# Pixie8888/R3DFSSeg

Measured on NVIDIA B200. Metric: MPTI episodes/s (2-way 5-shot, 2048 pts), higher is better.
Workload: dtype f32

## Files before the change

### r3dfsseg_b200/csrc/common.cuh

```cuda
#pragma once
#include <cuda_runtime.h>
#include <stdint.h>
#include <math.h>

#include "../../include/r3dfs.h"

#define R3DFS_FEAT_DIM 192
#define R3DFS_EC_WIDTH 64

extern thread_local long long r3dfs_launches;

#ifdef R3DFS_AB_SWITCHES
#include <stdlib.h>
#define R3DFS_GETENV(name) getenv(name)
#else
#define R3DFS_GETENV(name) ((const char*)nullptr)
#endif

#define R3DFS_CHECK_LAUNCH()                       \
  do {                                             \
    cudaError_t e__ = cudaGetLastError();          \
    if (e__ != cudaSuccess) return (int)e__;       \
    ++r3dfs_launches;                              \
  } while (0)
// ... 6 lines not shown
};

#define R3DFS_TRY(expr)                            \
  do {                                             \
    int rc__ = (expr);                             \
    if (rc__ != 0) return rc__;                    \
  } while (0)

static inline size_t align_up(size_t x, size_t a) { return (x + a - 1) / a * a; }

__host__ __device__ inline int lp_rowcap(int k) { return ((2 * k + 3) & ~3) + 4; }
__host__ __device__ inline int64_t lp_pack_groups(int64_t nn, int k) {
  return (nn * (int64_t)(2 * k) * 2 / 5 + 64 * nn + 63) / 64 * 64;
}
static inline size_t lp_solver_scratch_bytes(size_t G, size_t nn, int k) {
  return G * 16 * (4 + 32 * 3 * 2 + 3 * 1024 * 2) * 4 + 256 + 4 * G * (1 + nn) + 256 +
         (8 + 16) * G * (size_t)lp_pack_groups(nn, k) + 512;
}

struct WsBump {
  char* base;
  size_t cap;
  size_t off;
  __host__ WsBump(void* p, size_t c) : base((char*)p), cap(c), off(0) {}
  template <typename T>
  __host__ T* take(size_t n) {
    off = align_up(off, 256);
    T* r = (T*)(base + off);
    off += n * sizeof(T);
    return r;
  }
  __host__ bool ok() const { return off <= cap; }
// ... 92 lines not shown
```

### r3dfsseg_b200/csrc/lp.cu

```cuda
#include <cooperative_groups.h>

#include <stdlib.h>

#include "common.cuh"
#include "lp.cuh"

namespace cg = cooperative_groups;

#define GD_BM 128
#define GD_BN 64
#define GD_BK 16

template <int ROWS, int KC>
__device__ __forceinline__ void lp_load_tile_T(float* __restrict__ dst,
                                               const float* __restrict__ src, int ld, int64_t row0,
                                               int64_t rows_end, int k0, int k_end) {
  constexpr int KG = KC / 8;
  constexpr int PAIRS = (ROWS / 4) * KG;
  const int lane = threadIdx.x & 31, w = threadIdx.x >> 5;
  const int nw = blockDim.x >> 5;
  const int r_lo = lane & 3, k_lo = lane >> 2;
  for (int p = w; p < PAIRS; p += nw) {
    int kg = p % KG, rg = p / KG;
    int row = 4 * rg + r_lo, kk = 8 * kg + k_lo;
// ... 754 lines not shown
#pragma unroll
  for (int r = 0; r < 8; ++r) {
    const int t = 32 * r + lane;
    if (t < L) {
      src[t] = key[r];
      val[t] = w[r];
    }
  }
}

__global__ __launch_bounds__(256) void merge_rows_kernel(
    const int32_t* __restrict__ nbr, const float* __restrict__ sim,
    const int32_t* __restrict__ in_ptr, const int32_t* __restrict__ in_src,
    const float* __restrict__ in_w, const uint8_t* __restrict__ valid, int nn, int k,
    int32_t* __restrict__ cursor, int32_t* __restrict__ rowptr, int32_t* __restrict__ rowlen,
    uint16_t* __restrict__ mcol, float* __restrict__ mval) {
  extern __shared__ __align__(16) unsigned char s_raw[];
  const int g = blockIdx.y, wi = threadIdx.x >> 5, lane = threadIdx.x & 31;
  const int i = blockIdx.x * 8 + wi;
  int* s_idx = reinterpret_cast<int*>(s_raw) + wi * k;
  float* s_val = reinterpret_cast<float*>(s_raw) + 8 * k + wi * k;
  if (i >= nn) return;
  const int64_t vb = (int64_t)g * nn;
  if (!valid[vb + i]) {
    if (lane == 0) {
      rowptr[vb + i] = 0;
      rowlen[vb + i] = 0;
    }
    return;
  }
  const int64_t ob = (vb + i) * k;
  for (int t = lane; t < k; t += 32) {
    s_idx[t] = nbr[ob + t];
    s_val[t] = sim[ob + t];
  }
  __syncwarp();
  const int32_t* ptr = in_ptr + (int64_t)g * (nn + 1);
  const int64_t ib = vb * k;
  const int e0 = ptr[i], e1 = ptr[i + 1];
  int keep = 0;
  for (int t0 = e0; t0 < e1; t0 += 32) {
    const int t = t0 + lane;
// ... 4 lines not shown
      while (lo < hi) {
        const int mid = (lo + hi) >> 1;
        if (s_idx[mid] < s) lo = mid + 1; else hi = mid;
      }
      kp = !(lo < k && s_idx[lo] == s);
    }
    keep += __popc(__ballot_sync(0xffffffffu, kp));
  }
  const int total = k + keep;
  const int padded = (total + 3) & ~3;
  int start = 0;
  if (lane == 0) start = atomicAdd(&cursor[g], padded);
  start = __shfl_sync(0xffffffffu, start, 0);
  const int64_t mb = vb * lp_rowcap(k) + start;
  int run = 0;
  for (int t0 = e0; t0 < e1; t0 += 32) {
    const int t = t0 + lane;
    bool kp = false;
    int s = 0;
    float wv = 0.f;
    if (t < e1) {
      s = in_src[ib + t];
      wv = in_w[ib + t];
      int lo = 0, hi = k;
      while (lo < hi) {
        const int mid = (lo + hi) >> 1;
        if (s_idx[mid] < s) lo = mid + 1; else hi = mid;
      }
      if (lo < k && s_idx[lo] == s) s_val[lo] += wv; else kp = true;
    }
    const unsigned bal = __ballot_sync(0xffffffffu, kp);
    if (kp) {
      const int pos = k + run + __popc(bal & ((1u << lane) - 1));
      mcol[mb + pos] = (uint16_t)s;
      mval[mb + pos] = wv;
    }
    run += __popc(bal);
  }
  __syncwarp();
  for (int t = lane; t < k; t += 32) {
    mcol[mb + t] = (uint16_t)s_idx[t];
    mval[mb + t] = s_val[t];
  }
  if (lane < padded - total) {
    mcol[mb + total + lane] = 0;
    mval[mb + total + lane] = 0.f;
  }
  if (lane == 0) {
    rowptr[vb + i] = start;
    rowlen[vb + i] = total;
  }
}

__global__ __launch_bounds__(256) void degree_merged_kernel(const int32_t* __restrict__ rowptr,
                                                            const int32_t* __restrict__ rowlen,
                                                            const float* __restrict__ mval, int nn,
                                                            int k, float* __restrict__ dinv) {
  const int g = blockIdx.y;
  const int i = blockIdx.x * 8 + (threadIdx.x >> 5);
  if (i >= nn) return;
  const int lane = threadIdx.x & 31;
  const int64_t vb = (int64_t)g * nn;
  const int L = rowlen[vb + i];
  float d = 0.f;
  if (L > 0) {
    const float* v = mval + vb * lp_rowcap(k) + rowptr[vb + i];
    for (int t = lane; t < L; t += 32) d += v[t];
    d = warp_sum(d);
    d = sqrtf(1.0f / (d + 2.220446049250313e-16f));
  }
  if (lane == 0) dinv[vb + i] = d;
}

__global__ void normalize_merged_kernel(const int32_t* __restrict__ rowptr,
                                        const int32_t* __restrict__ rowlen,
                                        const uint16_t* __restrict__ mcol, float* __restrict__ mval,
                                        const float* __restrict__ dinv, int nn, int k) {
  const int g = blockIdx.y;
  const int i = blockIdx.x * 8 + (threadIdx.x >> 5);
  if (i >= nn) return;
  const int lane = threadIdx.x & 31;
  const int64_t vb = (int64_t)g * nn;
  const int L = rowlen[vb + i];
  const float* dg = dinv + vb;
  const float di = dg[i];
  const int64_t mb = vb * lp_rowcap(k) + rowptr[vb + i];
  for (int t = lane; t < L; t += 32) mval[mb + t] = (di * mval[mb + t]) * dg[mcol[mb + t]];
}

#define CG_THREADS 1024
#define CGC_MAXT 1024
#define CG_CL_MAX 16
#define CG_MAXC 8
#define CG_MAXPASS 3
#define CG_SEGR 48
#define CG_MAXPART 1024
#define CG_TAB_HDR 4
#define CG_TAB_INTS (CG_TAB_HDR + 32 * CG_MAXPASS * 2 + CG_MAXPASS * CGC_MAXT * 2)
#define CG_PK_SMEM (4096 * 4 + 8192 * 4 * 2)

struct CgExchange {
  float slot[2][CG_CL_MAX][CG_MAXC];
};

template <int NCV>
__device__ __forceinline__ void cg_allreduce(cg::cluster_group& cluster, CgExchange* ex,
                                             float* s_warp, const float* part, int& xcnt,
                                             float* total) {
  const int tid = threadIdx.x, lane = tid & 31, w = tid >> 5;
  const int rank = cluster.block_rank(), CL = cluster.num_blocks();
  const int n_warps = blockDim.x >> 5;
  float v[NCV];
#pragma unroll
// ... 10 lines not shown
    for (int r = 0; r < CL; ++r) {
      float* dst = cluster.map_shared_rank(&ex->slot[par][rank][tid], r);
      *dst = s;
    }
  }
  cluster.sync();
#pragma unroll
  for (int c = 0; c < NCV; ++c) {
    float s = 0.f;
    for (int r = 0; r < CL; ++r) s += ex->slot[par][r][c];
    total[c] = s;
  }
  ++xcnt;
}

__global__ __launch_bounds__(256) void cg_hist_kernel(const int32_t* __restrict__ rowptr,
                                                      const int32_t* __restrict__ rowlen,
                                                      const uint8_t* __restrict__ valid,
                                                      const uint16_t* __restrict__ mcol, int nn,
                                                      int k, int32_t* __restrict__ rowmax) {
  const int g = blockIdx.y;
  const int i = blockIdx.x * 8 + (threadIdx.x >> 5);
  if (i >= nn) return;
  const int lane = threadIdx.x & 31;
  const int64_t vb = (int64_t)g * nn;
  int mx = 0;
  if (valid[vb + i]) {
    const int L = rowlen[vb + i];
    const uint16_t* c = mcol + vb * lp_rowcap(k) + rowptr[vb + i];
    int cnt[8] = {0, 0, 0, 0, 0, 0, 0, 0};
    for (int t0 = 0; t0 < L; t0 += 32) {
      const int t = t0 + lane;
      const int res = t < L ? (int)(c[t] & 7) : -1;
#pragma unroll
      for (int b = 0; b < 8; ++b) cnt[b] += __popc(__ballot_sync(0xffffffffu, res == b));
    }
#pragma unroll
    for (int b = 0; b < 8; ++b) mx = max(mx, cnt[b]);
  }
  if (lane == 0) rowmax[vb + i] = mx;
}

__global__ __launch_bounds__(1024) void cg_pack_kernel(
    const int32_t* __restrict__ rowptr, const int32_t* __restrict__ rowlen,
    const int32_t* __restrict__ rowmax, const uint16_t* __restrict__ mcol,
    const float* __restrict__ mval, int nn, int k, int64_t pk_cap, int32_t* __restrict__ tab_all,
    int32_t* __restrict__ flags, uint2* __restrict__ pcol, float4* __restrict__ pval) {
  extern __shared__ __align__(16) unsigned char pk_smem[];
  uint32_t* s_key = reinterpret_cast<uint32_t*>(pk_smem);
  int* s_pre = reinterpret_cast<int*>(s_key + 4096);
  int* s_prx = s_pre + 8192;
  __shared__ int s_scan[2][32];
  __shared__ int s_tot[2];
  __shared__ int s_rng[2];
  __shared__ int s_wtot[32], s_wbase[32];
  const int CL = gridDim.x, rank = blockIdx.x, g = blockIdx.y;
  const int tid = threadIdx.x, lane = tid & 31, w = tid >> 5;
  const int64_t vb = (int64_t)g * nn;
  const int32_t* rp = rowptr + vb;
  const int32_t* rl = rowlen + vb;
  const int32_t* rmx = rowmax + vb;
  const uint16_t* mc = mcol + vb * lp_rowcap(k);
  const float* mv = mval + vb * lp_rowcap(k);
  int32_t* tab = tab_all + (size_t)(g * CL + rank) * CG_TAB_INTS;
  for (int e = tid; e < CG_TAB_HDR + 32 * CG_MAXPASS * 2; e += 1024) tab[e] = 0;
  {
    int nseg[8], run = 0, runx = 0;
#pragma unroll
    for (int u = 0; u < 8; ++u) {
      const int i = tid * 8 + u;
      nseg[u] = i < nn ? (rmx[i] + CG_SEGR - 1) / CG_SEGR : 0;
      run += nseg[u];
      runx += nseg[u] > 1 ? nseg[u] : 0;
    }
    int inc = run, incx = runx;
#pragma unroll
    for (int o = 1; o < 32; o <<= 1) {
      const int a = __shfl_up_sync(0xffffffffu, inc, o), ax = __shfl_up_sync(0xffffffffu, incx, o);
      if (lane >= o) {
        inc += a;
        incx += ax;
      }
    }
    if (lane == 31) {
      s_scan[0][w] = inc;
      s_scan[1][w] = incx;
// ... 38 lines not shown
  const int NV = s_tot[0];
  for (int i = tid; i < nn; i += 1024) {
    const int owner = NV > 0 ? min(CL - 1, (int)((int64_t)s_pre[i] * CL / NV)) : (i * CL) / nn;
    if (owner == rank) {
      atomicMin(&s_rng[0], i);
      atomicMax(&s_rng[1], i + 1);
    }
  }
  __syncthreads();
  const int lo = min(s_rng[0], s_rng[1]), hi = s_rng[1];
  const int pre_lo = lo < nn ? s_pre[lo] : NV, prx_lo = lo < nn ? s_prx[lo] : s_tot[1];
  const int nv = (hi < nn ? s_pre[hi] : NV) - pre_lo;
  const int nx = (hi < nn ? s_prx[hi] : s_tot[1]) - prx_lo;
  const int passes = (nv + CGC_MAXT - 1) / CGC_MAXT;
  const int64_t share = pk_cap / CL;
  bool bad = passes > CG_MAXPASS || nx > CG_MAXPART || hi - lo > 8191;
  int npow = 32;
  while (npow < nv) npow <<= 1;
  if (!bad) {
    for (int i = tid; i < npow; i += 1024) s_key[i] = 0;
    __syncthreads();
    for (int i = lo + tid; i < hi; i += 1024) {
      const int mx = rmx[i];
      const int ns = (mx + CG_SEGR - 1) / CG_SEGR;
      if (ns > 255) bad = true;
      for (int sg = 0; sg < ns && sg < 256; ++sg) {
        const int ranks = min(CG_SEGR, mx - sg * CG_SEGR);
        s_key[s_pre[i] - pre_lo + sg] =
            ((uint32_t)(2 * ranks) << 21) | ((uint32_t)(i - lo) << 8) | (uint32_t)sg;
      }
    }
// ... 31 lines not shown
        run += s_wtot[q];
      }
      s_tot[0] = run;
    }
    __syncthreads();
    if (s_tot[0] > share) bad = true;
  }
  if (tid == 0) {
    tab[0] = lo;
    tab[1] = hi;
    tab[2] = bad ? 0 : passes;
    tab[3] = nx;
    if (bad) atomicOr(&flags[g], 1);
  }
  if (bad) return;
  for (int e = tid; e < CG_MAXPASS * CGC_MAXT; e += 1024) {
    const int p = e / CGC_MAXT, t = e % CGC_MAXT;
    const int i = p * CGC_MAXT + t;
    int m0 = -1, m1 = 0;
    if (p < passes && i < nv) {
      const uint32_t key = s_key[i];
      const int rloc = (int)((key >> 8) & 0x1fffu), sg = (int)(key & 0xffu);
      const int ns = (rmx[lo + rloc] + CG_SEGR - 1) / CG_SEGR;
      m0 = (rloc << 8) | sg;
      m1 = (ns << 16) | (ns > 1 ? s_prx[lo + rloc] - prx_lo : 0);
    }
    tab[CG_TAB_HDR + 32 * CG_MAXPASS * 2 + 2 * e + 0] = m0;
    tab[CG_TAB_HDR + 32 * CG_MAXPASS * 2 + 2 * e + 1] = m1;
  }
  uint2* gc = pcol + (int64_t)g * pk_cap + rank * share;
  float4* gv = pval + (int64_t)g * pk_cap + rank * share;
  int base = s_wbase[w];
  for (int p = 0; p < passes; ++p) {
    const int i0 = p * CGC_MAXT + w * 32;
    const int rounds = i0 < nv ? (int)(s_key[i0] >> 21) : 0;
    if (lane == 0) {
      tab[CG_TAB_HDR + (w * CG_MAXPASS + p) * 2 + 0] = (int)(rank * share) + base;
      tab[CG_TAB_HDR + (w * CG_MAXPASS + p) * 2 + 1] = rounds;
    }
    for (int r = 0; r < rounds; ++r) {
      const unsigned t0 = (unsigned)(lane + 4 * r);
      uint2 c2;
      c2.x = (t0 & 7u) | (((t0 + 1) & 7u) << 16);
      c2.y = ((t0 + 2) & 7u) | (((t0 + 3) & 7u) << 16);
      gc[base + r * 32 + lane] = c2;
      gv[base + r * 32 + lane] = make_float4(0.f, 0.f, 0.f, 0.f);
    }
    __syncwarp();
    uint16_t* c16 = reinterpret_cast<uint16_t*>(gc + base);
    float* v32 = reinterpret_cast<float*>(gv + base);
    int my_L = 0, my_ptr = 0, my_sg = 0;
    if (i0 + lane < nv) {
      const uint32_t key = s_key[i0 + lane];
      const int row = lo + (int)((key >> 8) & 0x1fffu);
      my_L = rl[row];
      my_ptr = rp[row];
      my_sg = (int)(key & 0xffu);
    }
    const int n_here = min(32, nv - i0);
    for (int l = 0; l < n_here; ++l) {
      const int L = __shfl_sync(0xffffffffu, my_L, l), sg = __shfl_sync(0xffffffffu, my_sg, l);
      const int ptr = __shfl_sync(0xffffffffu, my_ptr, l);
      const int r_lo = sg * CG_SEGR, r_hi = r_lo + CG_SEGR;
      const uint16_t* c = mc + ptr;
      const float* v = mv + ptr;
      int seen[8] = {0, 0, 0, 0, 0, 0, 0, 0};
      int col_n = lane < L ? (int)c[lane] : -1;
      float val_n = lane < L ? v[lane] : 0.f;
      for (int t0 = 0; t0 < L; t0 += 32) {
        const int col = col_n;
        const float val = val_n;
        const int tn = t0 + 32 + lane;
        col_n = tn < L ? (int)c[tn] : -1;
        val_n = tn < L ? v[tn] : 0.f;
        const int res = col >= 0 ? (col & 7) : -1;
        int rho = -1;
#pragma unroll
        for (int b = 0; b < 8; ++b) {
          const uint32_t m = __ballot_sync(0xffffffffu, res == b);
          if (res == b) rho = seen[b] + __popc(m & ((1u << lane) - 1));
          seen[b] += __popc(m);
        }
        if (rho >= r_lo && rho < r_hi) {
          const int step = 8 * (rho - r_lo) + ((res - l) & 7);
          const int64_t d = ((int64_t)(step >> 2) * 32 + l) * 4 + (step & 3);
          c16[d] = (uint16_t)col;
          v32[d] = val;
        }
        int done_all = 1;
#pragma unroll
        for (int b = 0; b < 8; ++b) done_all &= seen[b] >= r_hi;
        if (done_all) break;
      }
    }
    __syncwarp();
    base += rounds * 32;
  }
}

template <int NCV>
__global__ __launch_bounds__(CGC_MAXT, 1) void lp_cg_kernel(
    const int32_t* __restrict__ rowptr, const int32_t* __restrict__ rowlen,
    const uint16_t* __restrict__ mcol, const float* __restrict__ mval,
    const uint8_t* __restrict__ valid, int nn, int k,
    const float* __restrict__ Y, int nc, float alpha, float tol, int max_iter,
    float* __restrict__ Z, float* __restrict__ X, float* __restrict__ R, float* __restrict__ Pv,
    float* __restrict__ AP, int32_t* __restrict__ iters_out, float* __restrict__ resid_out,
    const int32_t* __restrict__ tab_all, const int32_t* __restrict__ flags,
    const uint2* __restrict__ pcol, const float4* __restrict__ pval, int64_t pk_cap) {
  cg::cluster_group cluster = cg::this_cluster();
  const int CL = cluster.num_blocks(), rank = cluster.block_rank();
// ... 217 lines not shown
    for (int c = 0; c < nc; ++c) Zg[(int64_t)row * nc + c] = Xg[(int64_t)row * NCV + c];
  }
  if (rank == 0 && tid == 0) {
    if (iters_out) iters_out[g] = it;
    if (resid_out) {
      float m = 0.f;
#pragma unroll
      for (int c = 0; c < NCV; ++c)
        if (bb[c] > 0.f) m = fmaxf(m, sqrtf(rs[c] / bb[c]));
      resid_out[g] = m;
    }
  }
  cluster.sync();
}

template <int NCV>
static int launch_cg(int CL, int G, size_t smem, cudaStream_t st, const int32_t* rowptr,
                     const int32_t* rowlen, const uint16_t* mcol, const float* mval,
                     const uint8_t* valid, int nn, int k, const float* Y, int nc,
                     float alpha, float tol, int max_iter, float* Z, float* X, float* R, float* P,
                     float* AP, int32_t* iters_out, float* resid_out, void* scratch,
                     size_t scratch_bytes) {
  cudaError_t e = cudaFuncSetAttribute(lp_cg_kernel<NCV>,
                                       cudaFuncAttributeMaxDynamicSharedMemorySize, 200 * 1024);
  if (e != cudaSuccess) return (int)e;
  if (CL > 8) {
    e = cudaFuncSetAttribute(lp_cg_kernel<NCV>, cudaFuncAttributeNonPortableClusterSizeAllowed, 1);
    if (e != cudaSuccess) return (int)e;
  }
  const int T = CGC_MAXT;
  smem += sizeof(float) * (size_t)CG_MAXPART * NCV;
  cudaLaunchConfig_t cfg = {};
  cfg.gridDim = dim3(CL, G, 1);
  cfg.blockDim = dim3(T, 1, 1);
  cfg.dynamicSmemBytes = smem;
  cfg.stream = st;
  cudaLaunchAttribute attr[1];
  attr[0].id = cudaLaunchAttributeClusterDimension;
  attr[0].val.clusterDim.x = CL;
  attr[0].val.clusterDim.y = 1;
  attr[0].val.clusterDim.z = 1;
  cfg.attrs = attr;
  cfg.numAttrs = 1;
  {
    int n_clusters = 0;
    e = cudaOccupancyMaxActiveClusters(&n_clusters, lp_cg_kernel<NCV>, &cfg);
    if (e != cudaSuccess || n_clusters < 1) {
      (void)cudaGetLastError();
      return -1000;
    }
  }
  const int64_t pk_cap = lp_pack_groups(nn, k);
  const size_t tab_bytes = align_up(sizeof(int32_t) * (size_t)G * CL * CG_TAB_INTS, 256);
  const size_t flg_bytes = align_up(sizeof(int32_t) * (size_t)G * (1 + nn), 256);
  const size_t col_bytes = align_up(sizeof(uint2) * (size_t)G * pk_cap, 256);
  const size_t val_bytes = align_up(sizeof(float4) * (size_t)G * pk_cap, 256);
  if (!scratch || scratch_bytes < tab_bytes + flg_bytes + col_bytes + val_bytes)
    return R3DFS_E_WORKSPACE;
  unsigned char* sp = reinterpret_cast<unsigned char*>(scratch);
  int32_t* tab = reinterpret_cast<int32_t*>(sp);
  int32_t* flags = reinterpret_cast<int32_t*>(sp + tab_bytes);
  uint2* pcol = reinterpret_cast<uint2*>(sp + tab_bytes + flg_bytes);
  float4* pval = reinterpret_cast<float4*>(sp + tab_bytes + flg_bytes + col_bytes);
  e = cudaMemsetAsync(flags, 0, sizeof(int32_t) * (size_t)G, st);
  if (e != cudaSuccess) return (int)e;
  e = cudaFuncSetAttribute(cg_pack_kernel, cudaFuncAttributeMaxDynamicSharedMemorySize, CG_PK_SMEM);
  if (e != cudaSuccess) return (int)e;
  int32_t* rowmax = flags + G;
  cg_hist_kernel<<<dim3((nn + 7) / 8, G), 256, 0, st>>>(rowptr, rowlen, valid, mcol, nn, k, rowmax);
  R3DFS_CHECK_LAUNCH();
  cg_pack_kernel<<<dim3(CL, G), 1024, CG_PK_SMEM, st>>>(rowptr, rowlen, rowmax, mcol, mval, nn, k,
                                                       pk_cap, tab, flags, pcol, pval);
  R3DFS_CHECK_LAUNCH();
  const int32_t* tabc = tab;
  const int32_t* flc = flags;
  const uint2* pc = pcol;
  const float4* pv = pval;
  e = cudaLaunchKernelEx(&cfg, lp_cg_kernel<NCV>, rowptr, rowlen, mcol, mval, valid, nn, k, Y, nc,
                         alpha, tol, max_iter, Z, X, R, P, AP, iters_out, resid_out, tabc, flc, pc,
                         pv, pk_cap);
  if (e != cudaSuccess) return (int)e;
  ++r3dfs_launches;
  return 0;
}

#define GCG_SLOT 8
#define GCG_MAX_GS 160

__device__ __forceinline__ unsigned ld_acquire_u32(const unsigned* p) {
  unsigned v;
  asm volatile("ld.acquire.gpu.global.u32 %0, [%1];" : "=r"(v) : "l"(p) : "memory");
  return v;
}

__device__ __forceinline__ void group_barrier(unsigned* cnt, unsigned& target, int GS) {
  __syncthreads();
  if (threadIdx.x == 0) {
    target += (unsigned)GS;
// ... 447 lines not shown
  if (sr) sr->mark(R3DFS_ST_SELECT, st);
  edge_sim_kernel<<<dim3((nn + 7) / 8, G), 256, 0, st>>>(F, graph_rows, row_off, nn, D, valid, nbr,
                                                        k, sigma, sim);
  R3DFS_CHECK_LAUNCH();
  if (sr) sr->mark(R3DFS_ST_SIM, st);
  return 0;
}

int launch_lp_solve(const int32_t* rowptr, const int32_t* rowlen, const uint16_t* mcol,
                    const float* mval, const uint8_t* valid, int G, int nn, int k, const float* Y,
                    int nc, float alpha, float tol, int max_iter, float* Z, float* X, float* R,
                    float* P, float* AP, int32_t* iters_out, float* resid_out, cudaStream_t st,
                    bool latency, void* scratch, size_t scratch_bytes) {
  if (nc > CG_MAXC || nc < 1 || nn > 8192) return R3DFS_E_UNSUPPORTED;
  const int ncv = nc <= 4 ? 4 : 8;
  const size_t smem_cg = sizeof(float) * (size_t)nn * ncv;
  if (smem_cg > 200 * 1024) return R3DFS_E_UNSUPPORTED;
  int rc = -1000;
  static const bool no_group = R3DFS_GETENV("R3DFS_CG_NOGROUP") != nullptr;
  if (latency && !no_group) {
    const size_t scratch_floats = (size_t)G * nn * ncv;
    rc = ncv == 4 ? launch_cg_group<4>(G, st, rowptr, rowlen, mcol, mval, valid, nn, k, Y, nc, alpha,
                                       tol, max_iter, Z, P, AP, scratch_floats, iters_out, resid_out)
                  : launch_cg_group<8>(G, st, rowptr, rowlen, mcol, mval, valid, nn, k, Y, nc, alpha,
                                       tol, max_iter, Z, P, AP, scratch_floats, iters_out, resid_out);
    if (rc == 0) return 0;
    if (rc != -1000) return rc;
  }
  static const int cl_first = [] {
    const char* e = R3DFS_GETENV("R3DFS_CG_CLUSTER");
    const int v = e ? atoi(e) : 0;
    return (v == 16 || v == 8 || v == 4 || v == 2) ? v : 0;
  }();
  int dev = 0, n_sm = 0;
  cudaGetDevice(&dev);
  cudaDeviceGetAttribute(&n_sm, cudaDevAttrMultiProcessorCount, dev);
  const int rows_cta_max = CGC_MAXT * CG_MAXPASS;
  const int cl_need = (nn + rows_cta_max - 1) / rows_cta_max;
  int cl_start = cl_first ? cl_first : (G <= 4 ? 16 : max(1, min(8, n_sm / G)));
  cl_start = max(cl_start, cl_need);
  for (int CL = cl_start; CL >= cl_need && CL >= 1 && rc == -1000;
       CL = (CL & (CL - 1)) ? (1 << (31 - __builtin_clz(CL))) : CL >> 1) {
    if (ncv == 4)
      rc = launch_cg<4>(CL, G, smem_cg, st, rowptr, rowlen, mcol, mval, valid, nn, k, Y, nc, alpha,
                        tol, max_iter, Z, X, R, P, AP, iters_out, resid_out, scratch, scratch_bytes);
    else
      rc = launch_cg<8>(CL, G, smem_cg, st, rowptr, rowlen, mcol, mval, valid, nn, k, Y, nc, alpha,
                        tol, max_iter, Z, X, R, P, AP, iters_out, resid_out, scratch, scratch_bytes);
  }
  if (rc != 0) return rc == -1000 ? R3DFS_E_UNSUPPORTED : rc;
  return 0;
}

int launch_label_propagate(const int32_t* nbr, float* sim, const uint8_t* valid, int G, int nn,
                           int k, const float* Y, int nc, float alpha, float tol, int max_iter,
                           int32_t* in_cnt, int32_t* in_ptr, int32_t* in_src, float* in_w,
                           float* dinv, int32_t* rowptr, int32_t* rowlen, int32_t* cursor,
                           uint16_t* mcol, float* mval, float* Z, float* X, float* R, float* P,
                           float* AP, int32_t* iters_out, float* resid_out, cudaStream_t st,
                           const StageRec* sr, void* scratch, size_t scratch_bytes, bool latency,
                           void* dense_scratch, int32_t* dense_info) {
  if (nc > CG_MAXC || nc < 1 || nn > 8192) return R3DFS_E_UNSUPPORTED;
  cudaError_t e;
  const int64_t edges = (int64_t)nn * k;
  dim3 ge((unsigned)((edges + 255) / 256), G);
  const int W = (nn + 31) / 32;
// ... 21 lines not shown
    R3DFS_CHECK_LAUNCH();
    in_scan_kernel<<<G, 1024, 0, st>>>(in_cnt, nn, in_ptr);
    R3DFS_CHECK_LAUNCH();
    in_fill_kernel<<<ge, 256, 0, st>>>(nbr, sim, valid, nn, k, in_ptr, in_cnt, in_src, in_w);
    R3DFS_CHECK_LAUNCH();
    e = cudaFuncSetAttribute(in_sort_kernel, cudaFuncAttributeMaxDynamicSharedMemorySize, 8 * 8192);
    if (e != cudaSuccess) return (int)e;
    in_sort_warp_kernel<<<dim3((nn + 7) / 8, G), 256, 0, st>>>(in_ptr, nn, k, in_src, in_w);
    R3DFS_CHECK_LAUNCH();
    in_sort_kernel<<<dim3(nn, G), 256, 8 * 1024, st>>>(in_ptr, nn, k, in_src, in_w, 256, 1024);
    R3DFS_CHECK_LAUNCH();
    in_sort_kernel<<<dim3(nn, G), 256, 8 * 8192, st>>>(in_ptr, nn, k, in_src, in_w, 1024, 8192);
    R3DFS_CHECK_LAUNCH();
  }
  dim3 gr((nn + 7) / 8, G);
  e = cudaMemsetAsync(cursor, 0, sizeof(int32_t) * (size_t)G, st);
  if (e != cudaSuccess) return (int)e;
  const size_t smem_m = (size_t)8 * k * 8;
  e = cudaFuncSetAttribute(merge_rows_kernel, cudaFuncAttributeMaxDynamicSharedMemorySize,
                           (int)smem_m);
  if (e != cudaSuccess) return (int)e;
  merge_rows_kernel<<<gr, 256, smem_m, st>>>(nbr, sim, in_ptr, in_src, in_w, valid, nn, k, cursor,
                                            rowptr, rowlen, mcol, mval);
  R3DFS_CHECK_LAUNCH();
  degree_merged_kernel<<<gr, 256, 0, st>>>(rowptr, rowlen, mval, nn, k, dinv);
  R3DFS_CHECK_LAUNCH();
  normalize_merged_kernel<<<gr, 256, 0, st>>>(rowptr, rowlen, mcol, mval, dinv, nn, k);
  R3DFS_CHECK_LAUNCH();
  if (sr) sr->mark(R3DFS_ST_SYM, st);

  if (dense_scratch) {
    R3DFS_TRY(launch_lp_cholesky_solve(rowptr, rowlen, mcol, mval, valid, G, nn, k, Y, nc, alpha, Z,
                                       dense_scratch, dense_info, st));
    if (sr) sr->mark(R3DFS_ST_CG, st);
    return 0;
  }
  R3DFS_TRY(launch_lp_solve(rowptr, rowlen, mcol, mval, valid, G, nn, k, Y, nc, alpha, tol, max_iter,
                            Z, X, R, P, AP, iters_out, resid_out, st, latency, scratch,
                            scratch_bytes));
  if (sr) sr->mark(R3DFS_ST_CG, st);
  return 0;
}

int launch_query_head(const float* Z, int G, int nn, int q_off, int nq, int nc, const int64_t* qy,
                      float* logits, float* loss, int32_t* pred, cudaStream_t st) {
  query_head_kernel<<<G, 1024, 0, st>>>(Z, nn, q_off, nq, nc, qy, logits, loss, pred);
  R3DFS_CHECK_LAUNCH();
  return 0;
}

int launch_confusion(const int32_t* pred, const int64_t* gt, const int32_t* class_slot, int E,
                     int n_way, int64_t pts, int n_slots, int64_t* counters, cudaStream_t st) {
  const int64_t total = (int64_t)E * pts;
  confusion_kernel<<<(unsigned)((total + 255) / 256), 256, 0, st>>>(
// ... 6 lines not shown
```

Measured before the change: 942.6.

## Fuse CG sparse-matrix packing into merge and normalize kernels

Computes the per-row residue histogram (rowmax) inside merge_rows_kernel, which removes the separate cg_hist pass. The cg_pack kernel is split into a table-only kernel, and the actual scatter of normalized values into the packed CG layout moves into normalize_merged_kernel, which removes a second read of mcol/mval. The CG plan is now built before merging so these steps can share the layout. The changes add scratch space for a per-row segment map, extra atomics-free scatter writes and padding fills, and more complex indexing that could break correctness on edge cases.

```diff
diff --git a/r3dfsseg_b200/csrc/common.cuh b/r3dfsseg_b200/csrc/common.cuh
--- a/r3dfsseg_b200/csrc/common.cuh
+++ b/r3dfsseg_b200/csrc/common.cuh
@@ -44,8 +44,8 @@
   return (nn * (int64_t)(2 * k) * 2 / 5 + 64 * nn + 63) / 64 * 64;
 }
 static inline size_t lp_solver_scratch_bytes(size_t G, size_t nn, int k) {
-  return G * 16 * (4 + 32 * 3 * 2 + 3 * 1024 * 2) * 4 + 256 + 4 * G * (1 + nn) + 256 +
-         (8 + 16) * G * (size_t)lp_pack_groups(nn, k) + 512;
+  return G * 16 * (4 + 32 * 3 * 2 + 3 * 1024 * 4) * 4 + 256 + 4 * G * (1 + nn) + 256 + 4 * G * nn +
+         256 + (8 + 16) * G * (size_t)lp_pack_groups(nn, k) + 512;
 }
 
 struct WsBump {
diff --git a/r3dfsseg_b200/csrc/lp.cu b/r3dfsseg_b200/csrc/lp.cu
--- a/r3dfsseg_b200/csrc/lp.cu
+++ b/r3dfsseg_b200/csrc/lp.cu
@@ -792,7 +792,7 @@
     const int32_t* __restrict__ in_ptr, const int32_t* __restrict__ in_src,
     const float* __restrict__ in_w, const uint8_t* __restrict__ valid, int nn, int k,
     int32_t* __restrict__ cursor, int32_t* __restrict__ rowptr, int32_t* __restrict__ rowlen,
-    uint16_t* __restrict__ mcol, float* __restrict__ mval) {
+    uint16_t* __restrict__ mcol, float* __restrict__ mval, int32_t* __restrict__ rowmax) {
   extern __shared__ __align__(16) unsigned char s_raw[];
   const int g = blockIdx.y, wi = threadIdx.x >> 5, lane = threadIdx.x & 31;
   const int i = blockIdx.x * 8 + wi;
@@ -804,6 +804,7 @@
     if (lane == 0) {
       rowptr[vb + i] = 0;
       rowlen[vb + i] = 0;
+      if (rowmax) rowmax[vb + i] = 0;
     }
     return;
   }
@@ -838,6 +839,11 @@
   start = __shfl_sync(0xffffffffu, start, 0);
   const int64_t mb = vb * lp_rowcap(k) + start;
   int run = 0;
+  int rcnt[8] = {0, 0, 0, 0, 0, 0, 0, 0};
+  auto count_res = [&](int col) {
+#pragma unroll
+    for (int b = 0; b < 8; ++b) rcnt[b] += (col & 7) == b;
+  };
   for (int t0 = e0; t0 < e1; t0 += 32) {
     const int t = t0 + lane;
     bool kp = false;
@@ -858,6 +864,7 @@
       const int pos = k + run + __popc(bal & ((1u << lane) - 1));
       mcol[mb + pos] = (uint16_t)s;
       mval[mb + pos] = wv;
+      count_res(s);
     }
     run += __popc(bal);
   }
@@ -865,14 +872,21 @@
   for (int t = lane; t < k; t += 32) {
     mcol[mb + t] = (uint16_t)s_idx[t];
     mval[mb + t] = s_val[t];
+    count_res(s_idx[t]);
   }
   if (lane < padded - total) {
     mcol[mb + total + lane] = 0;
     mval[mb + total + lane] = 0.f;
   }
+  int mx = 0;
+  if (rowmax) {
+#pragma unroll
+    for (int b = 0; b < 8; ++b) mx = max(mx, (int)__reduce_add_sync(0xffffffffu, (unsigned)rcnt[b]));
+  }
   if (lane == 0) {
     rowptr[vb + i] = start;
     rowlen[vb + i] = total;
+    if (rowmax) rowmax[vb + i] = mx;
   }
 }
 
@@ -896,22 +910,6 @@
   if (lane == 0) dinv[vb + i] = d;
 }
 
-__global__ void normalize_merged_kernel(const int32_t* __restrict__ rowptr,
-                                        const int32_t* __restrict__ rowlen,
-                                        const uint16_t* __restrict__ mcol, float* __restrict__ mval,
-                                        const float* __restrict__ dinv, int nn, int k) {
-  const int g = blockIdx.y;
-  const int i = blockIdx.x * 8 + (threadIdx.x >> 5);
-  if (i >= nn) return;
-  const int lane = threadIdx.x & 31;
-  const int64_t vb = (int64_t)g * nn;
-  const int L = rowlen[vb + i];
-  const float* dg = dinv + vb;
-  const float di = dg[i];
-  const int64_t mb = vb * lp_rowcap(k) + rowptr[vb + i];
-  for (int t = lane; t < L; t += 32) mval[mb + t] = (di * mval[mb + t]) * dg[mcol[mb + t]];
-}
-
 #define CG_THREADS 1024
 #define CGC_MAXT 1024
 #define CG_CL_MAX 16
@@ -920,7 +918,8 @@
 #define CG_SEGR 48
 #define CG_MAXPART 1024
 #define CG_TAB_HDR 4
-#define CG_TAB_INTS (CG_TAB_HDR + 32 * CG_MAXPASS * 2 + CG_MAXPASS * CGC_MAXT * 2)
+#define CG_TAB_SEG (CG_TAB_HDR + 32 * CG_MAXPASS * 2 + CG_MAXPASS * CGC_MAXT * 2)
+#define CG_TAB_INTS (CG_TAB_SEG + CG_MAXPASS * CGC_MAXT * 2)
 #define CG_PK_SMEM (4096 * 4 + 8192 * 4 * 2)
 
 struct CgExchange {
@@ -961,38 +960,13 @@
   ++xcnt;
 }
 
-__global__ __launch_bounds__(256) void cg_hist_kernel(const int32_t* __restrict__ rowptr,
-                                                      const int32_t* __restrict__ rowlen,
-                                                      const uint8_t* __restrict__ valid,
-                                                      const uint16_t* __restrict__ mcol, int nn,
-                                                      int k, int32_t* __restrict__ rowmax) {
-  const int g = blockIdx.y;
-  const int i = blockIdx.x * 8 + (threadIdx.x >> 5);
-  if (i >= nn) return;
-  const int lane = threadIdx.x & 31;
-  const int64_t vb = (int64_t)g * nn;
-  int mx = 0;
-  if (valid[vb + i]) {
-    const int L = rowlen[vb + i];
-    const uint16_t* c = mcol + vb * lp_rowcap(k) + rowptr[vb + i];
-    int cnt[8] = {0, 0, 0, 0, 0, 0, 0, 0};
-    for (int t0 = 0; t0 < L; t0 += 32) {
-      const int t = t0 + lane;
-      const int res = t < L ? (int)(c[t] & 7) : -1;
-#pragma unroll
-      for (int b = 0; b < 8; ++b) cnt[b] += __popc(__ballot_sync(0xffffffffu, res == b));
-    }
-#pragma unroll
-    for (int b = 0; b < 8; ++b) mx = max(mx, cnt[b]);
-  }
-  if (lane == 0) rowmax[vb + i] = mx;
-}
-
-__global__ __launch_bounds__(1024) void cg_pack_kernel(
-    const int32_t* __restrict__ rowptr, const int32_t* __restrict__ rowlen,
-    const int32_t* __restrict__ rowmax, const uint16_t* __restrict__ mcol,
-    const float* __restrict__ mval, int nn, int k, int64_t pk_cap, int32_t* __restrict__ tab_all,
-    int32_t* __restrict__ flags, uint2* __restrict__ pcol, float4* __restrict__ pval) {
+__global__ __launch_bounds__(1024) void cg_table_kernel(const int32_t* __restrict__ rowmax,
+                                                        const int32_t* __restrict__ rowlen, int nn,
+                                                        int64_t pk_cap, int32_t* __restrict__ tab_all,
+                                                        int32_t* __restrict__ flags,
+                                                        int32_t* __restrict__ rowseg,
+                                                        uint2* __restrict__ pcol,
+                                                        float4* __restrict__ pval) {
   extern __shared__ __align__(16) unsigned char pk_smem[];
   uint32_t* s_key = reinterpret_cast<uint32_t*>(pk_smem);
   int* s_pre = reinterpret_cast<int*>(s_key + 4096);
@@ -1001,14 +975,11 @@
   __shared__ int s_tot[2];
   __shared__ int s_rng[2];
   __shared__ int s_wtot[32], s_wbase[32];
+  __shared__ int s_slice[32][CG_MAXPASS][2];
   const int CL = gridDim.x, rank = blockIdx.x, g = blockIdx.y;
   const int tid = threadIdx.x, lane = tid & 31, w = tid >> 5;
   const int64_t vb = (int64_t)g * nn;
-  const int32_t* rp = rowptr + vb;
-  const int32_t* rl = rowlen + vb;
-  const int32_t* rmx = rowmax + vb;
-  const uint16_t* mc = mcol + vb * lp_rowcap(k);
-  const float* mv = mval + vb * lp_rowcap(k);
+  const int32_t* rmx = rowmax ? rowmax + vb : nullptr;
   int32_t* tab = tab_all + (size_t)(g * CL + rank) * CG_TAB_INTS;
   for (int e = tid; e < CG_TAB_HDR + 32 * CG_MAXPASS * 2; e += 1024) tab[e] = 0;
   {
@@ -1016,7 +987,7 @@
 #pragma unroll
     for (int u = 0; u < 8; ++u) {
       const int i = tid * 8 + u;
-      nseg[u] = i < nn ? (rmx[i] + CG_SEGR - 1) / CG_SEGR : 0;
+      nseg[u] = i >= nn ? 0 : rmx ? (rmx[i] + CG_SEGR - 1) / CG_SEGR : (rowlen[vb + i] > 0);
       run += nseg[u];
       runx += nseg[u] > 1 ? nseg[u] : 0;
     }
@@ -1085,7 +1056,7 @@
   const int nx = (hi < nn ? s_prx[hi] : s_tot[1]) - prx_lo;
   const int passes = (nv + CGC_MAXT - 1) / CGC_MAXT;
   const int64_t share = pk_cap / CL;
-  bool bad = passes > CG_MAXPASS || nx > CG_MAXPART || hi - lo > 8191;
+  bool bad = !rmx || passes > CG_MAXPASS || nx > CG_MAXPART || hi - lo > 8191;
   int npow = 32;
   while (npow < nv) npow <<= 1;
   if (!bad) {
@@ -1147,87 +1118,127 @@
     if (bad) atomicOr(&flags[g], 1);
   }
   if (bad) return;
+  if (tid < 32) {
+    int base = (int)(rank * share) + s_wbase[tid];
+    for (int p = 0; p < passes; ++p) {
+      const int i0 = p * CGC_MAXT + tid * 32;
+      const int rounds = i0 < nv ? (int)(s_key[i0] >> 21) : 0;
+      tab[CG_TAB_HDR + (tid * CG_MAXPASS + p) * 2 + 0] = base;
+      tab[CG_TAB_HDR + (tid * CG_MAXPASS + p) * 2 + 1] = rounds;
+      s_slice[tid][p][0] = base;
+      s_slice[tid][p][1] = rounds;
+      base += rounds * 32;
+    }
+  }
+  __syncthreads();
   for (int e = tid; e < CG_MAXPASS * CGC_MAXT; e += 1024) {
     const int p = e / CGC_MAXT, t = e % CGC_MAXT;
-    const int i = p * CGC_MAXT + t;
     int m0 = -1, m1 = 0;
-    if (p < passes && i < nv) {
-      const uint32_t key = s_key[i];
+    if (p < passes && e < nv) {
+      const uint32_t key = s_key[e];
       const int rloc = (int)((key >> 8) & 0x1fffu), sg = (int)(key & 0xffu);
       const int ns = (rmx[lo + rloc] + CG_SEGR - 1) / CG_SEGR;
       m0 = (rloc << 8) | sg;
       m1 = (ns << 16) | (ns > 1 ? s_prx[lo + rloc] - prx_lo : 0);
+      const int j = s_pre[lo + rloc] - pre_lo + sg;
+      tab[CG_TAB_SEG + 2 * j + 0] = s_slice[t >> 5][p][0];
+      tab[CG_TAB_SEG + 2 * j + 1] = (s_slice[t >> 5][p][1] << 5) | (t & 31);
     }
     tab[CG_TAB_HDR + 32 * CG_MAXPASS * 2 + 2 * e + 0] = m0;
     tab[CG_TAB_HDR + 32 * CG_MAXPASS * 2 + 2 * e + 1] = m1;
   }
-  uint2* gc = pcol + (int64_t)g * pk_cap + rank * share;
-  float4* gv = pval + (int64_t)g * pk_cap + rank * share;
-  int base = s_wbase[w];
-  for (int p = 0; p < passes; ++p) {
-    const int i0 = p * CGC_MAXT + w * 32;
-    const int rounds = i0 < nv ? (int)(s_key[i0] >> 21) : 0;
-    if (lane == 0) {
-      tab[CG_TAB_HDR + (w * CG_MAXPASS + p) * 2 + 0] = (int)(rank * share) + base;
-      tab[CG_TAB_HDR + (w * CG_MAXPASS + p) * 2 + 1] = rounds;
-    }
-    for (int r = 0; r < rounds; ++r) {
-      const unsigned t0 = (unsigned)(lane + 4 * r);
+  for (int i = lo + tid; i < hi; i += 1024) rowseg[vb + i] = (rank << 16) | (s_pre[i] - pre_lo);
+  if (nv & 31) {
+    const int i0 = nv & ~31, p = i0 / CGC_MAXT, ws = (i0 % CGC_MAXT) >> 5;
+    const int base = s_slice[ws][p][0], rounds = s_slice[ws][p][1];
+    const int n_here = nv - i0, n_pad = 32 - n_here;
+    uint2* gc = pcol + (int64_t)g * pk_cap;
+    float4* gv = pval + (int64_t)g * pk_cap;
+    for (int e = tid; e < rounds * n_pad; e += 1024) {
+      const int r = e / n_pad, l = n_here + e % n_pad;
+      const unsigned t0 = (unsigned)(l + 4 * r);
       uint2 c2;
       c2.x = (t0 & 7u) | (((t0 + 1) & 7u) << 16);
       c2.y = ((t0 + 2) & 7u) | (((t0 + 3) & 7u) << 16);
-      gc[base + r * 32 + lane] = c2;
-      gv[base + r * 32 + lane] = make_float4(0.f, 0.f, 0.f, 0.f);
-    }
-    __syncwarp();
-    uint16_t* c16 = reinterpret_cast<uint16_t*>(gc + base);
-    float* v32 = reinterpret_cast<float*>(gv + base);
-    int my_L = 0, my_ptr = 0, my_sg = 0;
-    if (i0 + lane < nv) {
-      const uint32_t key = s_key[i0 + lane];
-      const int row = lo + (int)((key >> 8) & 0x1fffu);
-      my_L = rl[row];
-      my_ptr = rp[row];
-      my_sg = (int)(key & 0xffu);
-    }
-    const int n_here = min(32, nv - i0);
-    for (int l = 0; l < n_here; ++l) {
-      const int L = __shfl_sync(0xffffffffu, my_L, l), sg = __shfl_sync(0xffffffffu, my_sg, l);
-      const int ptr = __shfl_sync(0xffffffffu, my_ptr, l);
-      const int r_lo = sg * CG_SEGR, r_hi = r_lo + CG_SEGR;
-      const uint16_t* c = mc + ptr;
-      const float* v = mv + ptr;
-      int seen[8] = {0, 0, 0, 0, 0, 0, 0, 0};
-      int col_n = lane < L ? (int)c[lane] : -1;
-      float val_n = lane < L ? v[lane] : 0.f;
-      for (int t0 = 0; t0 < L; t0 += 32) {
-        const int col = col_n;
-        const float val = val_n;
-        const int tn = t0 + 32 + lane;
-        col_n = tn < L ? (int)c[tn] : -1;
-        val_n = tn < L ? v[tn] : 0.f;
-        const int res = col >= 0 ? (col & 7) : -1;
-        int rho = -1;
-#pragma unroll
-        for (int b = 0; b < 8; ++b) {
-          const uint32_t m = __ballot_sync(0xffffffffu, res == b);
-          if (res == b) rho = seen[b] + __popc(m & ((1u << lane) - 1));
-          seen[b] += __popc(m);
-        }
-        if (rho >= r_lo && rho < r_hi) {
-          const int step = 8 * (rho - r_lo) + ((res - l) & 7);
-          const int64_t d = ((int64_t)(step >> 2) * 32 + l) * 4 + (step & 3);
-          c16[d] = (uint16_t)col;
-          v32[d] = val;
-        }
-        int done_all = 1;
-#pragma unroll
-        for (int b = 0; b < 8; ++b) done_all &= seen[b] >= r_hi;
-        if (done_all) break;
-      }
-    }
-    __syncwarp();
-    base += rounds * 32;
+      gc[base + r * 32 + l] = c2;
+      gv[base + r * 32 + l] = make_float4(0.f, 0.f, 0.f, 0.f);
+    }
+  }
+}
+
+__global__ __launch_bounds__(256) void normalize_merged_kernel(
+    const int32_t* __restrict__ rowptr, const int32_t* __restrict__ rowlen,
+    const uint16_t* __restrict__ mcol, float* __restrict__ mval, const float* __restrict__ dinv,
+    int nn, int k, const int32_t* __restrict__ tab_all, int CL, const int32_t* __restrict__ flags,
+    const int32_t* __restrict__ rowseg, int64_t pk_cap, uint2* __restrict__ pcol,
+    float4* __restrict__ pval) {
+  const int g = blockIdx.y;
+  const int i = blockIdx.x * 8 + (threadIdx.x >> 5);
+  if (i >= nn) return;
+  const int lane = threadIdx.x & 31;
+  const int64_t vb = (int64_t)g * nn;
+  const int L = rowlen[vb + i];
+  const float* dg = dinv + vb;
+  const float di = dg[i];
+  const int64_t mb = vb * lp_rowcap(k) + rowptr[vb + i];
+  if (!tab_all || L == 0 || flags[g] != 0) {
+    for (int t = lane; t < L; t += 32) mval[mb + t] = (di * mval[mb + t]) * dg[mcol[mb + t]];
+    return;
+  }
+  const int rs = rowseg[vb + i];
+  const int2* seg =
+      reinterpret_cast<const int2*>(tab_all + (size_t)(g * CL + (rs >> 16)) * CG_TAB_INTS + CG_TAB_SEG) +
+      (rs & 0xffff);
+  uint16_t* c16 = reinterpret_cast<uint16_t*>(pcol + (int64_t)g * pk_cap);
+  float* v32 = reinterpret_cast<float*>(pval + (int64_t)g * pk_cap);
+  int seen[8] = {0, 0, 0, 0, 0, 0, 0, 0};
+  for (int t0 = 0; t0 < L; t0 += 32) {
+    const int t = t0 + lane;
+    int col = -1;
+    float val = 0.f;
+    if (t < L) {
+      col = (int)mcol[mb + t];
+      val = (di * mval[mb + t]) * dg[col];
+      mval[mb + t] = val;
+    }
+    const int res = col >= 0 ? (col & 7) : -1;
+    int rho = -1;
+#pragma unroll
+    for (int b = 0; b < 8; ++b) {
+      const uint32_t m = __ballot_sync(0xffffffffu, res == b);
+      if (res == b) rho = seen[b] + __popc(m & ((1u << lane) - 1));
+      seen[b] += __popc(m);
+    }
+    if (col >= 0) {
+      const int sg = rho / CG_SEGR, r = rho - sg * CG_SEGR;
+      const int2 d = seg[sg];
+      const int l = d.y & 31;
+      const int step = 8 * r + ((res - l) & 7);
+      const int64_t o = ((int64_t)d.x + (step >> 2) * 32 + l) * 4 + (step & 3);
+      c16[o] = (uint16_t)col;
+      v32[o] = val;
+    }
+  }
+  int mx = 0, my_cnt = 0;
+#pragma unroll
+  for (int b = 0; b < 8; ++b) {
+    mx = max(mx, seen[b]);
+    if ((lane & 7) == b) my_cnt = seen[b];
+  }
+  const int ns = (mx + CG_SEGR - 1) / CG_SEGR;
+  for (int sg = 0; sg < ns; ++sg) {
+    const int2 d = seg[sg];
+    const int l = d.y & 31, steps = 4 * (d.y >> 5);
+    for (int s0 = 0; s0 < steps; s0 += 32) {
+      const int s = s0 + lane;
+      const int res = (l + s) & 7;
+      const int have = __shfl_sync(0xffffffffu, my_cnt, res);
+      if (s < steps && sg * CG_SEGR + (s >> 3) >= have) {
+        const int64_t o = ((int64_t)d.x + (s >> 2) * 32 + l) * 4 + (s & 3);
+        c16[o] = (uint16_t)res;
+        v32[o] = 0.f;
+      }
+    }
   }
 }
 
@@ -1475,74 +1486,150 @@
   cluster.sync();
 }
 
-template <int NCV>
-static int launch_cg(int CL, int G, size_t smem, cudaStream_t st, const int32_t* rowptr,
-                     const int32_t* rowlen, const uint16_t* mcol, const float* mval,
-                     const uint8_t* valid, int nn, int k, const float* Y, int nc,
-                     float alpha, float tol, int max_iter, float* Z, float* X, float* R, float* P,
-                     float* AP, int32_t* iters_out, float* resid_out, void* scratch,
-                     size_t scratch_bytes) {
-  cudaError_t e = cudaFuncSetAttribute(lp_cg_kernel<NCV>,
-                                       cudaFuncAttributeMaxDynamicSharedMemorySize, 200 * 1024);
-  if (e != cudaSuccess) return (int)e;
-  if (CL > 8) {
-    e = cudaFuncSetAttribute(lp_cg_kernel<NCV>, cudaFuncAttributeNonPortableClusterSizeAllowed, 1);
-    if (e != cudaSuccess) return (int)e;
-  }
-  const int T = CGC_MAXT;
-  smem += sizeof(float) * (size_t)CG_MAXPART * NCV;
+struct CgPlan {
+  int CL = 0, ncv = 4;
+  size_t smem = 0;
+  int32_t* tab = nullptr;
+  int32_t* flags = nullptr;
+  int32_t* rowmax = nullptr;
+  int32_t* rowseg = nullptr;
+  uint2* pcol = nullptr;
+  float4* pval = nullptr;
+  int64_t pk_cap = 0;
+};
+
+static cudaLaunchConfig_t cg_launch_config(int CL, int G, size_t smem, cudaStream_t st,
+                                           cudaLaunchAttribute* attr) {
   cudaLaunchConfig_t cfg = {};
   cfg.gridDim = dim3(CL, G, 1);
-  cfg.blockDim = dim3(T, 1, 1);
+  cfg.blockDim = dim3(CGC_MAXT, 1, 1);
   cfg.dynamicSmemBytes = smem;
   cfg.stream = st;
-  cudaLaunchAttribute attr[1];
   attr[0].id = cudaLaunchAttributeClusterDimension;
   attr[0].val.clusterDim.x = CL;
   attr[0].val.clusterDim.y = 1;
   attr[0].val.clusterDim.z = 1;
   cfg.attrs = attr;
   cfg.numAttrs = 1;
-  {
-    int n_clusters = 0;
-    e = cudaOccupancyMaxActiveClusters(&n_clusters, lp_cg_kernel<NCV>, &cfg);
-    if (e != cudaSuccess || n_clusters < 1) {
-      (void)cudaGetLastError();
-      return -1000;
-    }
-  }
-  const int64_t pk_cap = lp_pack_groups(nn, k);
-  const size_t tab_bytes = align_up(sizeof(int32_t) * (size_t)G * CL * CG_TAB_INTS, 256);
+  return cfg;
+}
+
+template <int NCV>
+static int cg_cluster_fits(int CL, size_t smem) {
+  cudaError_t e = cudaFuncSetAttribute(lp_cg_kernel<NCV>,
+                                       cudaFuncAttributeMaxDynamicSharedMemorySize, (int)smem);
+  if (e != cudaSuccess) return (int)e;
+  if (CL > 8) {
+    e = cudaFuncSetAttribute(lp_cg_kernel<NCV>, cudaFuncAttributeNonPortableClusterSizeAllowed, 1);
+    if (e != cudaSuccess) return (int)e;
+  }
+  cudaLaunchAttribute attr[1];
+  const cudaLaunchConfig_t cfg = cg_launch_config(CL, 1, smem, nullptr, attr);
+  int n_clusters = 0;
+  e = cudaOccupancyMaxActiveClusters(&n_clusters, lp_cg_kernel<NCV>, &cfg);
+  if (e != cudaSuccess || n_clusters < 1) {
+    (void)cudaGetLastError();
+    return -1000;
+  }
+  return 0;
+}
+
+static int cg_plan(int G, int nn, int k, int nc, bool packed, void* scratch, size_t scratch_bytes,
+                   cudaStream_t st, CgPlan& pl) {
+  pl = CgPlan{};
+  pl.ncv = nc <= 4 ? 4 : 8;
+  int dev = 0, n_sm = 0, optin = 0;
+  cudaGetDevice(&dev);
+  cudaDeviceGetAttribute(&n_sm, cudaDevAttrMultiProcessorCount, dev);
+  cudaDeviceGetAttribute(&optin, cudaDevAttrMaxSharedMemoryPerBlockOptin, dev);
+  cudaFuncAttributes fa;
+  cudaError_t e = pl.ncv == 4 ? cudaFuncGetAttributes(&fa, lp_cg_kernel<4>)
+                              : cudaFuncGetAttributes(&fa, lp_cg_kernel<8>);
+  if (e != cudaSuccess) return (int)e;
+  const size_t avail = (size_t)optin - fa.sharedSizeBytes;
+  const size_t p_bytes = sizeof(float) * (size_t)nn * pl.ncv;
+  const size_t split_bytes = sizeof(float) * (size_t)CG_MAXPART * pl.ncv;
+  if (p_bytes > avail) return R3DFS_E_UNSUPPORTED;
+  if (p_bytes + split_bytes > avail) packed = false;
+  pl.smem = p_bytes + (packed ? split_bytes : 0);
+  static const int cl_first = [] {
+    const char* ev = R3DFS_GETENV("R3DFS_CG_CLUSTER");
+    const int v = ev ? atoi(ev) : 0;
+    return (v == 16 || v == 8 || v == 4 || v == 2) ? v : 0;
+  }();
+  const int rows_cta_max = CGC_MAXT * CG_MAXPASS;
+  const int cl_need = (nn + rows_cta_max - 1) / rows_cta_max;
+  int cl_start = cl_first ? cl_first : (G <= 4 ? 16 : max(1, min(8, n_sm / G)));
+  cl_start = max(cl_start, cl_need);
+  int rc = -1000;
+  for (int CL = cl_start; CL >= cl_need && CL >= 1 && rc == -1000;
+       CL = (CL & (CL - 1)) ? (1 << (31 - __builtin_clz(CL))) : CL >> 1) {
+    rc = pl.ncv == 4 ? cg_cluster_fits<4>(CL, pl.smem) : cg_cluster_fits<8>(CL, pl.smem);
+    if (rc == 0) pl.CL = CL;
+  }
+  if (rc != 0) return rc == -1000 ? R3DFS_E_UNSUPPORTED : rc;
+  pl.pk_cap = lp_pack_groups(nn, k);
+  const size_t tab_bytes = align_up(sizeof(int32_t) * (size_t)G * pl.CL * CG_TAB_INTS, 256);
   const size_t flg_bytes = align_up(sizeof(int32_t) * (size_t)G * (1 + nn), 256);
-  const size_t col_bytes = align_up(sizeof(uint2) * (size_t)G * pk_cap, 256);
-  const size_t val_bytes = align_up(sizeof(float4) * (size_t)G * pk_cap, 256);
-  if (!scratch || scratch_bytes < tab_bytes + flg_bytes + col_bytes + val_bytes)
+  const size_t seg_bytes = align_up(sizeof(int32_t) * (size_t)G * nn, 256);
+  const size_t col_bytes = align_up(sizeof(uint2) * (size_t)G * pl.pk_cap, 256);
+  const size_t val_bytes = align_up(sizeof(float4) * (size_t)G * pl.pk_cap, 256);
+  if (!scratch || scratch_bytes < tab_bytes + flg_bytes + seg_bytes + col_bytes + val_bytes)
     return R3DFS_E_WORKSPACE;
   unsigned char* sp = reinterpret_cast<unsigned char*>(scratch);
-  int32_t* tab = reinterpret_cast<int32_t*>(sp);
-  int32_t* flags = reinterpret_cast<int32_t*>(sp + tab_bytes);
-  uint2* pcol = reinterpret_cast<uint2*>(sp + tab_bytes + flg_bytes);
-  float4* pval = reinterpret_cast<float4*>(sp + tab_bytes + flg_bytes + col_bytes);
-  e = cudaMemsetAsync(flags, 0, sizeof(int32_t) * (size_t)G, st);
+  pl.tab = reinterpret_cast<int32_t*>(sp);
+  pl.flags = reinterpret_cast<int32_t*>(sp + tab_bytes);
+  pl.rowmax = packed ? pl.flags + G : nullptr;
+  pl.rowseg = reinterpret_cast<int32_t*>(sp + tab_bytes + flg_bytes);
+  pl.pcol = reinterpret_cast<uint2*>(sp + tab_bytes + flg_bytes + seg_bytes);
+  pl.pval = reinterpret_cast<float4*>(sp + tab_bytes + flg_bytes + seg_bytes + col_bytes);
+  e = cudaMemsetAsync(pl.flags, 0, sizeof(int32_t) * (size_t)G, st);
   if (e != cudaSuccess) return (int)e;
-  e = cudaFuncSetAttribute(cg_pack_kernel, cudaFuncAttributeMaxDynamicSharedMemorySize, CG_PK_SMEM);
+  return 0;
+}
+
+static int launch_cg_table(const CgPlan& pl, const int32_t* rowlen, int G, int nn, cudaStream_t st) {
+  cudaError_t e =
+      cudaFuncSetAttribute(cg_table_kernel, cudaFuncAttributeMaxDynamicSharedMemorySize, CG_PK_SMEM);
   if (e != cudaSuccess) return (int)e;
-  int32_t* rowmax = flags + G;
-  cg_hist_kernel<<<dim3((nn + 7) / 8, G), 256, 0, st>>>(rowptr, rowlen, valid, mcol, nn, k, rowmax);
+  cg_table_kernel<<<dim3(pl.CL, G), 1024, CG_PK_SMEM, st>>>(pl.rowmax, rowlen, nn, pl.pk_cap, pl.tab,
+                                                           pl.flags, pl.rowseg, pl.pcol, pl.pval);
   R3DFS_CHECK_LAUNCH();
-  cg_pack_kernel<<<dim3(CL, G), 1024, CG_PK_SMEM, st>>>(rowptr, rowlen, rowmax, mcol, mval, nn, k,
-                                                       pk_cap, tab, flags, pcol, pval);
-  R3DFS_CHECK_LAUNCH();
-  const int32_t* tabc = tab;
-  const int32_t* flc = flags;
-  const uint2* pc = pcol;
-  const float4* pv = pval;
+  return 0;
+}
+
+template <int NCV>
+static int launch_cg(const CgPlan& pl, int G, cudaStream_t st, const int32_t* rowptr,
+                     const int32_t* rowlen, const uint16_t* mcol, const float* mval,
+                     const uint8_t* valid, int nn, int k, const float* Y, int nc, float alpha,
+                     float tol, int max_iter, float* Z, float* X, float* R, float* P, float* AP,
+                     int32_t* iters_out, float* resid_out) {
+  cudaError_t e = cudaFuncSetAttribute(lp_cg_kernel<NCV>,
+                                       cudaFuncAttributeMaxDynamicSharedMemorySize, (int)pl.smem);
+  if (e != cudaSuccess) return (int)e;
+  cudaLaunchAttribute attr[1];
+  const cudaLaunchConfig_t cfg = cg_launch_config(pl.CL, G, pl.smem, st, attr);
+  const int32_t* tabc = pl.tab;
+  const int32_t* flc = pl.flags;
+  const uint2* pc = pl.pcol;
+  const float4* pv = pl.pval;
   e = cudaLaunchKernelEx(&cfg, lp_cg_kernel<NCV>, rowptr, rowlen, mcol, mval, valid, nn, k, Y, nc,
                          alpha, tol, max_iter, Z, X, R, P, AP, iters_out, resid_out, tabc, flc, pc,
-                         pv, pk_cap);
+                         pv, pl.pk_cap);
   if (e != cudaSuccess) return (int)e;
   ++r3dfs_launches;
   return 0;
+}
+
+static int launch_cg_plan(const CgPlan& pl, int G, cudaStream_t st, const int32_t* rowptr,
+                          const int32_t* rowlen, const uint16_t* mcol, const float* mval,
+                          const uint8_t* valid, int nn, int k, const float* Y, int nc, float alpha,
+                          float tol, int max_iter, float* Z, float* X, float* R, float* P, float* AP,
+                          int32_t* iters_out, float* resid_out) {
+  return pl.ncv == 4 ? launch_cg<4>(pl, G, st, rowptr, rowlen, mcol, mval, valid, nn, k, Y, nc, alpha,
+                                    tol, max_iter, Z, X, R, P, AP, iters_out, resid_out)
+                     : launch_cg<8>(pl, G, st, rowptr, rowlen, mcol, mval, valid, nn, k, Y, nc, alpha,
+                                    tol, max_iter, Z, X, R, P, AP, iters_out, resid_out);
 }
 
 #define GCG_SLOT 8
@@ -2020,42 +2107,21 @@
                     bool latency, void* scratch, size_t scratch_bytes) {
   if (nc > CG_MAXC || nc < 1 || nn > 8192) return R3DFS_E_UNSUPPORTED;
   const int ncv = nc <= 4 ? 4 : 8;
-  const size_t smem_cg = sizeof(float) * (size_t)nn * ncv;
-  if (smem_cg > 200 * 1024) return R3DFS_E_UNSUPPORTED;
-  int rc = -1000;
   static const bool no_group = R3DFS_GETENV("R3DFS_CG_NOGROUP") != nullptr;
   if (latency && !no_group) {
     const size_t scratch_floats = (size_t)G * nn * ncv;
-    rc = ncv == 4 ? launch_cg_group<4>(G, st, rowptr, rowlen, mcol, mval, valid, nn, k, Y, nc, alpha,
-                                       tol, max_iter, Z, P, AP, scratch_floats, iters_out, resid_out)
-                  : launch_cg_group<8>(G, st, rowptr, rowlen, mcol, mval, valid, nn, k, Y, nc, alpha,
-                                       tol, max_iter, Z, P, AP, scratch_floats, iters_out, resid_out);
-    if (rc == 0) return 0;
+    const int rc =
+        ncv == 4 ? launch_cg_group<4>(G, st, rowptr, rowlen, mcol, mval, valid, nn, k, Y, nc, alpha,
+                                      tol, max_iter, Z, P, AP, scratch_floats, iters_out, resid_out)
+                 : launch_cg_group<8>(G, st, rowptr, rowlen, mcol, mval, valid, nn, k, Y, nc, alpha,
+                                      tol, max_iter, Z, P, AP, scratch_floats, iters_out, resid_out);
     if (rc != -1000) return rc;
   }
-  static const int cl_first = [] {
-    const char* e = R3DFS_GETENV("R3DFS_CG_CLUSTER");
-    const int v = e ? atoi(e) : 0;
-    return (v == 16 || v == 8 || v == 4 || v == 2) ? v : 0;
-  }();
-  int dev = 0, n_sm = 0;
-  cudaGetDevice(&dev);
-  cudaDeviceGetAttribute(&n_sm, cudaDevAttrMultiProcessorCount, dev);
-  const int rows_cta_max = CGC_MAXT * CG_MAXPASS;
-  const int cl_need = (nn + rows_cta_max - 1) / rows_cta_max;
-  int cl_start = cl_first ? cl_first : (G <= 4 ? 16 : max(1, min(8, n_sm / G)));
-  cl_start = max(cl_start, cl_need);
-  for (int CL = cl_start; CL >= cl_need && CL >= 1 && rc == -1000;
-       CL = (CL & (CL - 1)) ? (1 << (31 - __builtin_clz(CL))) : CL >> 1) {
-    if (ncv == 4)
-      rc = launch_cg<4>(CL, G, smem_cg, st, rowptr, rowlen, mcol, mval, valid, nn, k, Y, nc, alpha,
-                        tol, max_iter, Z, X, R, P, AP, iters_out, resid_out, scratch, scratch_bytes);
-    else
-      rc = launch_cg<8>(CL, G, smem_cg, st, rowptr, rowlen, mcol, mval, valid, nn, k, Y, nc, alpha,
-                        tol, max_iter, Z, X, R, P, AP, iters_out, resid_out, scratch, scratch_bytes);
-  }
-  if (rc != 0) return rc == -1000 ? R3DFS_E_UNSUPPORTED : rc;
-  return 0;
+  CgPlan pl;
+  R3DFS_TRY(cg_plan(G, nn, k, nc, false, scratch, scratch_bytes, st, pl));
+  R3DFS_TRY(launch_cg_table(pl, rowlen, G, nn, st));
+  return launch_cg_plan(pl, G, st, rowptr, rowlen, mcol, mval, valid, nn, k, Y, nc, alpha, tol,
+                        max_iter, Z, X, R, P, AP, iters_out, resid_out);
 }
 
 int launch_label_propagate(const int32_t* nbr, float* sim, const uint8_t* valid, int G, int nn,
@@ -2107,6 +2173,9 @@
     R3DFS_CHECK_LAUNCH();
   }
   dim3 gr((nn + 7) / 8, G);
+  const bool cluster = !dense_scratch && !latency;
+  CgPlan pl;
+  if (cluster) R3DFS_TRY(cg_plan(G, nn, k, nc, true, scratch, scratch_bytes, st, pl));
   e = cudaMemsetAsync(cursor, 0, sizeof(int32_t) * (size_t)G, st);
   if (e != cudaSuccess) return (int)e;
   const size_t smem_m = (size_t)8 * k * 8;
@@ -2114,11 +2183,14 @@
                            (int)smem_m);
   if (e != cudaSuccess) return (int)e;
   merge_rows_kernel<<<gr, 256, smem_m, st>>>(nbr, sim, in_ptr, in_src, in_w, valid, nn, k, cursor,
-                                            rowptr, rowlen, mcol, mval);
+                                            rowptr, rowlen, mcol, mval, pl.rowmax);
   R3DFS_CHECK_LAUNCH();
+  if (cluster) R3DFS_TRY(launch_cg_table(pl, rowlen, G, nn, st));
   degree_merged_kernel<<<gr, 256, 0, st>>>(rowptr, rowlen, mval, nn, k, dinv);
   R3DFS_CHECK_LAUNCH();
-  normalize_merged_kernel<<<gr, 256, 0, st>>>(rowptr, rowlen, mcol, mval, dinv, nn, k);
+  normalize_merged_kernel<<<gr, 256, 0, st>>>(rowptr, rowlen, mcol, mval, dinv, nn, k,
+                                              pl.rowmax ? pl.tab : nullptr, pl.CL,
+                                              pl.flags, pl.rowseg, pl.pk_cap, pl.pcol, pl.pval);
   R3DFS_CHECK_LAUNCH();
   if (sr) sr->mark(R3DFS_ST_SYM, st);
 
@@ -2128,9 +2200,13 @@
     if (sr) sr->mark(R3DFS_ST_CG, st);
     return 0;
   }
-  R3DFS_TRY(launch_lp_solve(rowptr, rowlen, mcol, mval, valid, G, nn, k, Y, nc, alpha, tol, max_iter,
-                            Z, X, R, P, AP, iters_out, resid_out, st, latency, scratch,
-                            scratch_bytes));
+  if (cluster)
+    R3DFS_TRY(launch_cg_plan(pl, G, st, rowptr, rowlen, mcol, mval, valid, nn, k, Y, nc, alpha, tol,
+                             max_iter, Z, X, R, P, AP, iters_out, resid_out));
+  else
+    R3DFS_TRY(launch_lp_solve(rowptr, rowlen, mcol, mval, valid, G, nn, k, Y, nc, alpha, tol,
+                              max_iter, Z, X, R, P, AP, iters_out, resid_out, st, latency, scratch,
+                              scratch_bytes));
   if (sr) sr->mark(R3DFS_ST_CG, st);
   return 0;
 }
```

Result: faster. 952.1 (median of 6 runs) (+1.0%).
